# abargum/RAVE

Hardware: AMD Instinct MI355X
Metric: audio samples/sec/GPU (48 kHz v2 encode+decode); × real-time factor (higher is better)
Workload: dtype fp32 (per conv / fused unit the faster of exact-fp32 MFMA and fp32 on the bf16 matrix cores: operands split exactly into 3 bf16 parts (24 significand bits), 6 of the 9 cross products (the 3 dropped are each < 2^-25 |a b|), fp32 accumulate; edges exact-fp32 MFMA); 1 GPU; v2 non-causal encode+decode, 16 x 65536 samples per GPU (BASELINE configs[1]); global_batch=16, samples_per_clip=65536, parallelism=dp1 (batch shards, RCCL all-gather of latents)

## Files before the change

### include/rave_amd.h

```cpp
#ifndef RAVE_AMD_H
#define RAVE_AMD_H

#include <stddef.h>
#include <stdint.h>

#ifdef __cplusplus
extern "C" {
#endif

#define RAVE_ABI_VERSION 21
#define RAVE_SPLITK_TICKETS 4096
#define RAVE_SPLITK_STATUS_WORD (RAVE_SPLITK_TICKETS - 1)

enum {
    RAVE_OK = 0,
    RAVE_ERR_ARG = -1,
    RAVE_ERR_HIP = -2,
    RAVE_ERR_UNSUPPORTED = -3,
    RAVE_ERR_STATE = -4,
    RAVE_ERR_COOP = -5
};

enum { RAVE_ACT_NONE = 0, RAVE_ACT_LEAKY = 1, RAVE_ACT_SNAKE = 2 };

// ... 167 lines not shown

typedef struct rave_noise_backward_args {
    int32_t batch, frames, n_band, noise_bands;
    int32_t target, _pad0;
    const float* amp; int64_t a_sb, a_sc;
    const float* u;   int64_t u_sb;
    const float* gy;  int64_t gy_sb, gy_sc;
    float* gamp;      int64_t ga_sb, ga_sc;
} rave_noise_backward_args;
int rave_noise_synth_backward(const rave_noise_backward_args* a, void* stream);

typedef struct rave_adain_args {
    int32_t batch, channels, t_len, mode;
    int32_t max_batch, row0;
    const float* x; int64_t x_sb, x_sc;
    float* y;       int64_t y_sb, y_sc;
    float* stats;
    float* counters;
    uint32_t* ticket;
} rave_adain_args;
int rave_adain(const rave_adain_args* a, void* stream);

typedef struct rave_adain_backward_args {
    int32_t batch, channels, t_len, mode;
    int32_t max_batch, row0;
    const float* gy; int64_t gy_sb, gy_sc;
    float* gx;       int64_t gx_sb, gx_sc;
    const float* stats;
    const float* counters;
} rave_adain_backward_args;
int rave_adain_backward(const rave_adain_backward_args* a, void* stream);

typedef struct rave_unit_args {
    int32_t channels, batch, t_len, dilation;
    int32_t pad_left, act;
    float leaky_slope; int32_t precision;
    const float* x; int64_t x_sb, x_sc;
    float* y;       int64_t y_sb, y_sc;
    const float* weight;
    const float* bias1; const float* bias2;
    const float* alpha0; const float* alpha2;
    float* workspace;
    uint32_t* status;
    int32_t x_len;
    int32_t res_shift;
    int32_t coop_rb;
    int32_t reserved0;
} rave_unit_args;
int64_t rave_unit_packed_size(int channels);
int rave_unit_pack_weight(const float* w1, const float* w2, int channels, float* packed);
int64_t rave_unit_split_packed_size(int channels);
int rave_unit_split_pack_weight(const float* w1, const float* w2, int channels, float* packed);
int rave_unit_ring_pack_weight(const float* w1, const float* w2, int channels, float* packed);
int64_t rave_unit_bf3_packed_size(int channels);
int rave_unit_bf3_pack_weight(const float* w1, const float* w2, int channels, float* packed);
int64_t rave_unit_workspace(const rave_unit_args* a);
int rave_residual_unit(const rave_unit_args* a, void* stream);
int rave_debug_coop(int64_t spin_limit, int force_giveup);

#define RAVE_STACK_UNITS 3
typedef struct rave_stack_args {
    int32_t channels, batch, t_len, act;
    float leaky_slope; int32_t precision;
    int32_t dilation[RAVE_STACK_UNITS], pad_left[RAVE_STACK_UNITS];
    const float* x; int64_t x_sb, x_sc;
    float* y;       int64_t y_sb, y_sc;
    const float* weight[RAVE_STACK_UNITS];
    const float* bias1[RAVE_STACK_UNITS];
    const float* bias2[RAVE_STACK_UNITS];
    const float* alpha0[RAVE_STACK_UNITS];
    const float* alpha2[RAVE_STACK_UNITS];
} rave_stack_args;
int rave_stack_supported(int channels);
int rave_residual_stack(const rave_stack_args* a, void* stream);

typedef struct rave_edge_args {
    int32_t batch, frames;
    int32_t conv_c_in, conv_c_out, conv_kernel, conv_pad_left;
    int32_t pqmf_taps, pqmf_pad_left;
    int32_t mode, act;
    float leaky_slope;
    int32_t fill_channels, fill_t;
    int32_t precision;
    const float* x;     int64_t x_sb, x_sc;
    float* y;           int64_t y_sb, y_sc;
    const float* weight;
    const float* bias;
    const float* alpha;
    const float* filter;
    const float* noise; int64_t n_sb, n_sc;
    float* fill_y;      int64_t f_sb, f_sc;
    const float* fill_values;
    int64_t fill_vs;
} rave_edge_args;
int rave_encoder_head(const rave_edge_args* a, void* stream);
int rave_decoder_tail(const rave_edge_args* a, void* stream);
#define RAVE_EDGE_FILTER_FLOATS 8836
int rave_encoder_head_pack_filter(const float* hkf, int n_band, int taps, int n_out_bands, float* image);
int rave_decoder_tail_pack_filter(const float* hki, int n_band, int taps, float* image);
int rave_encoder_head_pack_filter_f32(const float* hkf, int n_band, int taps, int n_out_bands, float* image);
int rave_decoder_tail_pack_filter_f32(const float* hki, int n_band, int taps, float* image);

enum {
    RAVE_OP_CONV = 1,
    RAVE_OP_PQMF_ANALYSIS = 2,
    RAVE_OP_PQMF_SYNTHESIS = 3,
    RAVE_OP_FILL = 4,
    RAVE_OP_RVQ_ENCODE = 5,
    RAVE_OP_RVQ_DECODE = 6,
    RAVE_OP_SHIFT_HISTORY = 7,
    RAVE_OP_COPY = 8,
    RAVE_OP_NOISE = 9,
    RAVE_OP_ADAIN = 10,
    RAVE_OP_UNIT = 11,
    RAVE_OP_STACK = 12,
    RAVE_OP_HEAD = 13,
    RAVE_OP_TAIL = 14
};

#define RAVE_OP_PAYLOAD 240
typedef struct rave_plan_op {
    int32_t kind, _pad0;
    union {
        rave_conv1d_args conv;
        rave_pqmf_analysis_args ana;
        rave_pqmf_synthesis_args syn;
        rave_fill_args fill;
        rave_rvq_args rvq;
        rave_shift_args shift;
        rave_copy_args copy;
        rave_noise_args noise;
        rave_adain_args adain;
        rave_unit_args unit;
        rave_stack_args stack;
        rave_edge_args edge;
        unsigned char raw[RAVE_OP_PAYLOAD];
    } u;
} rave_plan_op;

typedef struct rave_reloc {
    int32_t op, field_offset, slot, _pad0;
    int64_t byte_offset;
} rave_reloc;

typedef struct rave_plan rave_plan;
int rave_plan_create(const rave_plan_op* ops, int n_ops, const rave_reloc* relocs, int n_relocs,
                     rave_plan** out);
int rave_plan_run(rave_plan* plan, void* const* slots, int n_slots, void* stream);
int rave_plan_destroy(rave_plan* plan);
int rave_plan_size(const rave_plan* plan);
int rave_plan_profile(rave_plan* plan, int enable);
int rave_plan_op_times(rave_plan* plan, float* ms, int n);

int rave_fill_uniform(float* y, int64_t n, uint64_t seed, float lo, float hi, void* stream);

typedef struct rave_fir_args {
    int32_t batch, t_in, t_out, phases, taps, stride, pad_left, _pad0;
    const float* x; int64_t x_sb;
    float* y;       int64_t y_sb;
    const float* h;
} rave_fir_args;
int rave_fir(const rave_fir_args* a, void* stream);

typedef struct rave_row_stats_args {
    int32_t batch, channels, t_len, act;
    float leaky_slope, var_min, var_max, _pad0;
    const float* x; int64_t x_sb, x_sc;
    float* y;       int64_t y_sb;
} rave_row_stats_args;
int rave_row_stats(const rave_row_stats_args* a, void* stream);

typedef struct rave_attn_pool_args {
    int32_t batch, channels, t_len, act;
    float leaky_slope, var_min, var_max, _pad0;
    const float* x;      int64_t x_sb, x_sc;
    const float* logits; int64_t l_sb, l_sc;
    float* y;            int64_t y_sb;
// ... 196 lines not shown
```

### rave_amd/_native.py

```python
from __future__ import annotations

import ctypes as C
import os

_HERE = os.path.dirname(os.path.abspath(__file__))
LIB_PATH = os.path.join(_HERE, "librave_amd.so")
if os.environ.get("RAVE_AMD_DIAG_LIB") == "1":
    LIB_PATH = os.path.join(_HERE, "librave_amd_diag.so")
if os.environ.get("RAVE_AMD_LIB_VARIANT"):
    LIB_PATH = os.path.join(_HERE, f"librave_amd_{os.environ['RAVE_AMD_LIB_VARIANT']}.so")

RAVE_OK = 0
RAVE_ERR_ARG = -1
RAVE_ERR_HIP = -2
RAVE_ERR_UNSUPPORTED = -3
RAVE_ERR_STATE = -4
RAVE_ERR_COOP = -5

ACT = {"none": 0, "leaky": 1, "snake": 2}

OP_CONV = 1
OP_PQMF_ANALYSIS = 2
OP_PQMF_SYNTHESIS = 3
OP_FILL = 4
# ... 121 lines not shown


class AdainArgs(C.Structure):
    _fields_ = [("batch", i32), ("channels", i32), ("t_len", i32), ("mode", i32),
                ("max_batch", i32), ("row0", i32),
                ("x", vp), ("x_sb", i64), ("x_sc", i64),
                ("y", vp), ("y_sb", i64), ("y_sc", i64),
                ("stats", vp), ("counters", vp), ("ticket", vp)]


class NoiseBackwardArgs(C.Structure):
    _fields_ = [("batch", i32), ("frames", i32), ("n_band", i32), ("noise_bands", i32),
                ("target", i32), ("_pad0", i32),
                ("amp", vp), ("a_sb", i64), ("a_sc", i64),
                ("u", vp), ("u_sb", i64),
                ("gy", vp), ("gy_sb", i64), ("gy_sc", i64),
                ("gamp", vp), ("ga_sb", i64), ("ga_sc", i64)]


class AdainBackwardArgs(C.Structure):
    _fields_ = [("batch", i32), ("channels", i32), ("t_len", i32), ("mode", i32),
                ("max_batch", i32), ("row0", i32),
                ("gy", vp), ("gy_sb", i64), ("gy_sc", i64),
                ("gx", vp), ("gx_sb", i64), ("gx_sc", i64),
                ("stats", vp), ("counters", vp)]


class UnitArgs(C.Structure):
    _fields_ = [("channels", i32), ("batch", i32), ("t_len", i32), ("dilation", i32),
                ("pad_left", i32), ("act", i32), ("leaky_slope", f32), ("precision", i32),
                ("x", vp), ("x_sb", i64), ("x_sc", i64),
                ("y", vp), ("y_sb", i64), ("y_sc", i64),
                ("weight", vp), ("bias1", vp), ("bias2", vp), ("alpha0", vp), ("alpha2", vp),
                ("workspace", vp), ("status", vp), ("x_len", i32), ("res_shift", i32),
                ("coop_rb", i32), ("reserved0", i32)]


STACK_UNITS = 3


class StackArgs(C.Structure):
    _fields_ = ([("channels", i32), ("batch", i32), ("t_len", i32), ("act", i32),
                 ("leaky_slope", f32), ("precision", i32)]
                + [(f"dilation{u}", i32) for u in range(STACK_UNITS)]
                + [(f"pad_left{u}", i32) for u in range(STACK_UNITS)]
                + [("x", vp), ("x_sb", i64), ("x_sc", i64), ("y", vp), ("y_sb", i64), ("y_sc", i64)]
                + [(f"{f}{u}", vp) for f in ("weight", "bias1", "bias2", "alpha0", "alpha2")
                   for u in range(STACK_UNITS)])


class FirArgs(C.Structure):
    _fields_ = [("batch", i32), ("t_in", i32), ("t_out", i32), ("phases", i32), ("taps", i32),
                ("stride", i32), ("pad_left", i32), ("_pad0", i32),
                ("x", vp), ("x_sb", i64), ("y", vp), ("y_sb", i64), ("h", vp)]


class RowStatsArgs(C.Structure):
    _fields_ = [("batch", i32), ("channels", i32), ("t_len", i32), ("act", i32),
                ("leaky_slope", f32), ("var_min", f32), ("var_max", f32), ("_pad0", i32),
                ("x", vp), ("x_sb", i64), ("x_sc", i64), ("y", vp), ("y_sb", i64)]


class AttnPoolArgs(C.Structure):
    _fields_ = [("batch", i32), ("channels", i32), ("t_len", i32), ("act", i32),
                ("leaky_slope", f32), ("var_min", f32), ("var_max", f32), ("_pad0", i32),
                ("x", vp), ("x_sb", i64), ("x_sc", i64), ("logits", vp), ("l_sb", i64), ("l_sc", i64),
                ("y", vp), ("y_sb", i64)]


class LinearArgs(C.Structure):
    _fields_ = [("batch", i32), ("n_in", i32), ("n_out", i32), ("_pad0", i32),
                ("x", vp), ("x_sb", i64), ("w", vp), ("bias", vp), ("y", vp), ("y_sb", i64)]


class MaxPoolArgs(C.Structure):
    _fields_ = [("batch", i32), ("channels", i32), ("t_out", i32), ("kernel", i32),
                ("x", vp), ("x_sb", i64), ("x_sc", i64), ("y", vp), ("y_sb", i64), ("y_sc", i64)]


class EdgeArgs(C.Structure):
    _fields_ = [("batch", i32), ("frames", i32), ("conv_c_in", i32), ("conv_c_out", i32), ("conv_kernel", i32),
                ("conv_pad_left", i32), ("pqmf_taps", i32), ("pqmf_pad_left", i32), ("mode", i32), ("act", i32),
                ("leaky_slope", f32), ("fill_channels", i32), ("fill_t", i32), ("precision", i32),
                ("x", vp), ("x_sb", i64), ("x_sc", i64), ("y", vp), ("y_sb", i64), ("y_sc", i64),
                ("weight", vp), ("bias", vp), ("alpha", vp), ("filter", vp),
                ("noise", vp), ("n_sb", i64), ("n_sc", i64),
                ("fill_y", vp), ("f_sb", i64), ("f_sc", i64), ("fill_values", vp), ("fill_vs", i64)]


STFT_MAX_SCALES = 8


class StftArgs(C.Structure):
    _fields_ = [("rows", i32), ("t_len", i32), ("n", i32), ("_pad0", i32),
                ("x", vp), ("table", vp), ("y", vp)]


class DistanceArgs(C.Structure):
    _fields_ = [("rows", i32), ("t_len", i32), ("n_scales", i32), ("log_epsilon", f32),
                ("scales", i32 * STFT_MAX_SCALES),
                ("x", vp), ("y", vp), ("tables", vp * STFT_MAX_SCALES),
                ("workspace", vp), ("out", vp)]


STFT_LOSS_V1, STFT_LOSS_MULTIRES = 0, 1


class StftLossArgs(C.Structure):
    _fields_ = [("rows", i32), ("t_len", i32), ("n_res", i32), ("kind", i32),
                ("n_fft", i32 * STFT_MAX_SCALES), ("hop", i32 * STFT_MAX_SCALES), ("win", i32 * STFT_MAX_SCALES),
                ("log_epsilon", f32), ("_pad0", i32),
                ("tables", vp * STFT_MAX_SCALES), ("target", vp), ("value", vp),
                ("workspace", vp), ("out", vp), ("saved", vp), ("grad_out", vp), ("grad_value", vp)]


class YinArgs(C.Structure):
    _fields_ = [("rows", i32), ("t_len", i32), ("sample_rate", i32), ("_pad0", i32),
                ("pitch_min", C.c_double), ("pitch_max", C.c_double),
                ("frame_stride", C.c_double), ("threshold", C.c_double),
                ("x_sr", i64), ("x", vp), ("f0", vp), ("cmdf", vp)]


class F0OneHotArgs(C.Structure):
    _fields_ = [("batch", i32), ("frames", i32), ("bins", i32), ("_pad0", i32),
                ("log_lo", f32), ("log_span", f32),
                ("y_sb", i64), ("y_sc", i64), ("f0", vp), ("y", vp)]


MAX_RATIOS = 8
MAX_DILATIONS = 8


class ModelConfig(C.Structure):
    _fields_ = [("n_band", i32), ("enc_bands", i32), ("capacity", i32), ("latent_size", i32),
                ("kernel_size", i32), ("speaker_size", i32), ("n_ratios", i32),
                ("ratios", i32 * MAX_RATIOS), ("n_dilations", i32 * MAX_RATIOS),
                ("dilations", (i32 * MAX_DILATIONS) * MAX_RATIOS),
                ("amplitude_modulation", i32), ("causal", i32), ("activation", i32), ("adain", i32),
                ("leaky_slope", f32), ("conv_bias", i32), ("convt_bias", i32),
                ("noise", i32), ("noise_hidden", i32), ("noise_bands", i32), ("n_noise_ratios", i32),
                ("noise_ratios", i32 * MAX_RATIOS), ("rvq_quantizers", i32), ("rvq_codebook_size", i32),
                ("fuse_units", i32), ("speaker_rows", i32)]


class Param(C.Structure):
    _fields_ = [("name", C.c_char_p), ("data", vp), ("numel", i64)]


class OpInfo(C.Structure):
    _fields_ = [("kind", i32), ("precision", i32), ("flops", C.c_double), ("bytes", C.c_double),
                ("label", C.c_char * 96)]


PAYLOAD = 240


class PlanOp(C.Structure):
    _fields_ = [("kind", i32), ("_pad0", i32), ("raw", C.c_ubyte * PAYLOAD)]


class Reloc(C.Structure):
    _fields_ = [("op", i32), ("field_offset", i32), ("slot", i32), ("_pad0", i32),
                ("byte_offset", i64)]


STRUCTS = [ConvArgs, AnalysisArgs, SynthesisArgs, FillArgs, RvqArgs, ShiftArgs, PlanOp, Reloc,
           CopyArgs, NoiseArgs, AdainArgs, UnitArgs, StackArgs, ModelConfig, Param, OpInfo,
           FirArgs, RowStatsArgs, AttnPoolArgs, LinearArgs, MaxPoolArgs, EdgeArgs,
           StftArgs, DistanceArgs, YinArgs, F0OneHotArgs, SynthesisBackwardArgs, AnalysisBackwardArgs,
           ConvBackwardArgs, NoiseBackwardArgs, AdainBackwardArgs, StftLossArgs]

EXPORTS = [
    "rave_last_error", "rave_abi_version", "rave_struct_sizes",
    "rave_conv1d_chunk", "rave_conv1d_packed_size", "rave_conv1d_pack_weight", "rave_conv1d_pack_weight_device",
    "rave_conv1d",
    "rave_conv1d_workspace", "rave_conv1d_backward_workspace", "rave_conv1d_backward_data",
    "rave_conv1d_backward_weight", "rave_conv_transpose1d_backward_workspace", "rave_conv_transpose1d_backward_data",
    "rave_conv_transpose1d_backward_weight", "rave_conv1d_configs", "rave_conv1d_split_packed_size", "rave_conv1d_split_pack_weight",
    "rave_conv1d_ring_pack_weight", "rave_conv1d_bf3_packed_size", "rave_conv1d_bf3_pack_weight",
    "rave_pqmf_analysis", "rave_pqmf_synthesis", "rave_pqmf_analysis_backward", "rave_pqmf_synthesis_backward",
    "rave_fill_channels", "rave_copy",
    "rave_rvq_workspace", "rave_rvq_encode", "rave_rvq_decode", "rave_shift_history", "rave_noise_synth", "rave_adain",
    "rave_noise_synth_backward", "rave_adain_backward",
    "rave_unit_packed_size", "rave_unit_pack_weight", "rave_residual_unit",
    "rave_unit_split_packed_size", "rave_unit_split_pack_weight", "rave_unit_ring_pack_weight",
    "rave_unit_bf3_packed_size", "rave_unit_bf3_pack_weight",
    "rave_unit_workspace", "rave_debug_coop", "rave_model_check",
    "rave_stack_supported", "rave_residual_stack",
    "rave_plan_create", "rave_plan_run", "rave_plan_destroy", "rave_plan_size",
    "rave_plan_profile", "rave_plan_op_times", "rave_fill_uniform",
    "rave_model_param_count", "rave_model_param_info", "rave_model_create", "rave_model_destroy",
    "rave_model_encode", "rave_model_decode", "rave_model_forward", "rave_model_encode_codes",
    "rave_model_decode_codes", "rave_model_noise_shape", "rave_model_adain_control", "rave_model_set_row0",
    "rave_model_set_speaker", "rave_model_set_speakers", "rave_model_set_speaker_row0", "rave_model_speaker_info",
    "rave_model_adain_count", "rave_model_adain_info", "rave_model_adain_get", "rave_model_adain_set",
    "rave_model_tuning_get", "rave_model_tuning_set", "rave_model_plan_ops", "rave_model_profile",
    "rave_model_op_times", "rave_stream_create", "rave_stream_destroy", "rave_stream_reset",
    "rave_stream_encode", "rave_stream_decode", "rave_stream_encode_codes", "rave_stream_decode_codes",
    "rave_stream_delay",
    "rave_stream_launches",
    "rave_fir", "rave_row_stats", "rave_attn_pool", "rave_linear", "rave_maxpool",
    "rave_encoder_head", "rave_decoder_tail", "rave_encoder_head_pack_filter", "rave_decoder_tail_pack_filter",
    "rave_encoder_head_pack_filter_f32", "rave_decoder_tail_pack_filter_f32",
    "rave_stft_table_size", "rave_stft_pack_table", "rave_stft_mag",
    "rave_audio_distance_workspace", "rave_audio_distance",
    "rave_yin_shape", "rave_yin", "rave_f0_onehot", "rave_pitch_onehot",
    "rave_stft_loss_table_size", "rave_stft_loss_pack_table", "rave_stft_loss_workspace",
    "rave_stft_loss_forward", "rave_stft_loss_backward",
]
EDGE_FILTER_FLOATS = 8836


class NativeError(RuntimeError):
    pass


def _load():
    if not os.path.exists(LIB_PATH):
        raise ImportError(f"rave_amd native library not built: {LIB_PATH} is missing "
                          "(run `python -c 'import __graft_entry__ as g; g.build()'` or "
                          "`make -C rave_amd/csrc`)")
    lib = C.CDLL(LIB_PATH)
    lib.rave_last_error.restype = C.c_char_p
    lib.rave_abi_version.restype = C.c_int
    lib.rave_struct_sizes.argtypes = [C.POINTER(i64), C.c_int]
    lib.rave_conv1d_chunk.argtypes = [C.c_int] * 5
    lib.rave_conv1d_packed_size.argtypes = [C.c_int] * 6
    lib.rave_conv1d_packed_size.restype = i64
    lib.rave_conv1d_pack_weight.argtypes = [vp] + [C.c_int] * 7 + [vp]
    lib.rave_conv1d_pack_weight_device.argtypes = [vp] + [C.c_int] * 7 + [vp, vp]
    lib.rave_conv1d_workspace.argtypes = [C.POINTER(ConvArgs)]
    lib.rave_conv1d_configs.argtypes = [C.POINTER(ConvArgs), C.POINTER(i32), C.c_int]
    lib.rave_conv1d_split_packed_size.argtypes = [C.c_int] * 6
    lib.rave_conv1d_split_packed_size.restype = i64
    lib.rave_conv1d_split_pack_weight.argtypes = [vp] + [C.c_int] * 7 + [vp]
    lib.rave_conv1d_ring_pack_weight.argtypes = [vp] + [C.c_int] * 7 + [vp]
    lib.rave_conv1d_bf3_packed_size.argtypes = [C.c_int] * 6
    lib.rave_conv1d_bf3_packed_size.restype = i64
    lib.rave_conv1d_bf3_pack_weight.argtypes = [vp] + [C.c_int] * 7 + [vp]
    lib.rave_encoder_head_pack_filter.argtypes = [vp, C.c_int, C.c_int, C.c_int, vp]
    lib.rave_encoder_head_pack_filter_f32.argtypes = [vp, C.c_int, C.c_int, C.c_int, vp]
    lib.rave_decoder_tail_pack_filter_f32.argtypes = [vp, C.c_int, C.c_int, vp]
    lib.rave_decoder_tail_pack_filter.argtypes = [vp, C.c_int, C.c_int, vp]
    lib.rave_unit_packed_size.argtypes = [C.c_int]
    lib.rave_unit_packed_size.restype = i64
    lib.rave_unit_pack_weight.argtypes = [vp, vp, C.c_int, vp]
    lib.rave_unit_workspace.argtypes = [C.c_void_p]
    lib.rave_unit_workspace.restype = i64
    lib.rave_debug_coop.argtypes = [i64, C.c_int]
    lib.rave_unit_split_packed_size.argtypes = [C.c_int]
    lib.rave_stack_supported.argtypes = [C.c_int]
    lib.rave_unit_split_packed_size.restype = i64
    lib.rave_unit_split_pack_weight.argtypes = [vp, vp, C.c_int, vp]
    lib.rave_unit_ring_pack_weight.argtypes = [vp, vp, C.c_int, vp]
    lib.rave_unit_bf3_packed_size.argtypes = [C.c_int]
    lib.rave_unit_bf3_packed_size.restype = i64
    lib.rave_unit_bf3_pack_weight.argtypes = [vp, vp, C.c_int, vp]
    lib.rave_conv1d_workspace.restype = i64
    lib.rave_conv1d_backward_workspace.argtypes = [C.POINTER(ConvBackwardArgs)]
    lib.rave_conv1d_backward_workspace.restype = i64
    lib.rave_conv_transpose1d_backward_workspace.argtypes = [C.POINTER(ConvBackwardArgs)]
    lib.rave_conv_transpose1d_backward_workspace.restype = i64
    lib.rave_rvq_workspace.argtypes = [C.POINTER(RvqArgs)]
    lib.rave_rvq_workspace.restype = i64
    for name, st in [("rave_conv1d", ConvArgs), ("rave_pqmf_analysis", AnalysisArgs),
                     ("rave_pqmf_synthesis", SynthesisArgs), ("rave_fill_channels", FillArgs),
                     ("rave_pqmf_synthesis_backward", SynthesisBackwardArgs),
                     ("rave_pqmf_analysis_backward", AnalysisBackwardArgs),
                     ("rave_conv1d_backward_data", ConvBackwardArgs),
                     ("rave_conv1d_backward_weight", ConvBackwardArgs),
                     ("rave_conv_transpose1d_backward_data", ConvBackwardArgs),
                     ("rave_conv_transpose1d_backward_weight", ConvBackwardArgs),
                     ("rave_rvq_encode", RvqArgs), ("rave_rvq_decode", RvqArgs),
                     ("rave_shift_history", ShiftArgs), ("rave_copy", CopyArgs),
                     ("rave_noise_synth", NoiseArgs), ("rave_adain", AdainArgs),
                     ("rave_noise_synth_backward", NoiseBackwardArgs), ("rave_adain_backward", AdainBackwardArgs),
                     ("rave_residual_unit", UnitArgs), ("rave_residual_stack", StackArgs),
                     ("rave_fir", FirArgs), ("rave_row_stats", RowStatsArgs), ("rave_attn_pool", AttnPoolArgs),
                     ("rave_linear", LinearArgs), ("rave_maxpool", MaxPoolArgs),
                     ("rave_encoder_head", EdgeArgs), ("rave_decoder_tail", EdgeArgs)]:
        getattr(lib, name).argtypes = [C.POINTER(st), vp]
    lib.rave_stft_table_size.argtypes = [C.c_int]
    lib.rave_stft_table_size.restype = i64
    lib.rave_stft_pack_table.argtypes = [C.c_int, vp]
    lib.rave_stft_mag.argtypes = [C.POINTER(StftArgs), vp]
    lib.rave_audio_distance_workspace.argtypes = [C.POINTER(DistanceArgs)]
    lib.rave_audio_distance_workspace.restype = i64
    lib.rave_audio_distance.argtypes = [C.POINTER(DistanceArgs), vp]
    lib.rave_stft_loss_table_size.argtypes = [C.c_int, C.c_int]
    lib.rave_stft_loss_table_size.restype = i64
    lib.rave_stft_loss_pack_table.argtypes = [C.c_int, C.c_int, vp]
    lib.rave_stft_loss_workspace.argtypes = [C.POINTER(StftLossArgs)]
    lib.rave_stft_loss_workspace.restype = i64
# ... 222 lines not shown
```

### rave_amd/csrc/edge_split.hip

```cpp
#include "common.h"
#include "pack_shared.h"

#include <algorithm>
#include <cmath>

namespace rave {

typedef _Float16 e_h8 __attribute__((ext_vector_type(8)));
typedef _Float16 e_h4 __attribute__((ext_vector_type(4)));
typedef float e_f32x4 __attribute__((ext_vector_type(4)));
typedef float e_f32x16 __attribute__((ext_vector_type(16)));
typedef float e_f32x8 __attribute__((ext_vector_type(8)));
typedef __bf16 e_b8 __attribute__((ext_vector_type(8)));
typedef __bf16 e_b4 __attribute__((ext_vector_type(4)));

__device__ __forceinline__ e_f32x8 e_ld8(const float* p) {
    const e_f32x4 u = *reinterpret_cast<const e_f32x4*>(p), v = *reinterpret_cast<const e_f32x4*>(p + 4);
    return e_f32x8{u[0], u[1], u[2], u[3], v[0], v[1], v[2], v[3]};
}

constexpr int kEdgeWaves = 8;
constexpr int kEdgeNT = 64 * kEdgeWaves;
constexpr int kEdgeK7 = 7;
constexpr int kEdgeKW = 544;
constexpr int kEdgeFP = 552;
constexpr int kSynTapsE = 33;
constexpr int kAnaTapsE = 513;

constexpr int kEdgeFilterHalves = 2 * 16 * kEdgeFP;
constexpr int kEdgeFilterFloats = kEdgeFilterHalves / 2 + 4;

struct EdgeGeo {
    int tiles;
    int w_mb;
    int w_bytes;
    int y_vec;
    int64_t w_frag_floats;
};

__device__ __forceinline__ void e_split(float v, _Float16& hi, _Float16& lo) {
    hi = (_Float16)v;
    lo = (_Float16)((v - (float)hi) * 2048.0f);
}

struct EdgeW {
    __amdgpu_buffer_rsrc_t rs;
    int mb_count;
    int np = 2;
    __device__ unsigned off(int chunk, int mb, int tap, int plane, int lane) const {
        return (unsigned)((((chunk * mb_count + mb) * kEdgeK7 + tap) * np + plane) * 1024 + lane * 16);
    }
    __device__ e_h8 frag(int chunk, int mb, int tap, int plane, int lane) const {
        return __builtin_bit_cast(e_h8, __builtin_amdgcn_raw_buffer_load_b128(rs, off(chunk, mb, tap, plane, lane), 0, 0));
    }
    __device__ static e_f32x8 f32(const e_h8& p0, const e_h8& p1) {
        const e_f32x4 u = __builtin_bit_cast(e_f32x4, p0), v = __builtin_bit_cast(e_f32x4, p1);
        return e_f32x8{u[0], u[1], u[2], u[3], v[0], v[1], v[2], v[3]};
    }
};

#ifdef RAVE_EDGE_STOP
#define EDGE_STOP(n, v)                                                   \
    if (RAVE_EDGE_STOP == (n)) {                                          \
        if (threadIdx.x == 0) a.y[(int64_t)blockIdx.x] = (float)(v);      \
        return;                                                           \
    }
#else
#define EDGE_STOP(n, v)
#endif

constexpr int kHF = 256;
constexpr int kHAB = kHF / 32 + 1;
constexpr int kHBR = 32 * kHAB;
constexpr int kHBP = 24;
constexpr int kHXS = 512 * (kHAB - 1) + 32 * 15 + kEdgeKW;
__host__ __device__ constexpr int e_xi(int i) { return i + 8 * (i >> 7); }
constexpr int kHXP = e_xi(kHXS) + 8;
constexpr int kHeadLds = (2 * 16 * kEdgeFP + 2 * kHXP + 2 * kHBR * kHBP) * 2 + 4 * kEdgeWaves * 4 + 16 +
                         kEdgeWaves * 64 * 4 * 4;
constexpr int kHeadBaBand = (3 * 16 * kEdgeFP + 3 * kHXP) * 2;
static_assert(kHeadBaBand % 16 == 0, "band planes 16-byte aligned");
constexpr int kHeadLdsBa = kHeadBaBand + kHBR * kHBP * 4 + 4 * kEdgeWaves * 4 + 16 + kEdgeWaves * 64 * 4 * 4;

template <int AR>
__global__ __launch_bounds__(kEdgeNT) void encoder_head_kernel(rave_edge_args a, EdgeGeo geo) {
    constexpr bool FC = AR != 0;
    constexpr bool F32 = AR == 1, BA = AR == 2;
// ... 245 lines not shown
    const int MB = (a.conv_c_out + 31) / 32;
    e_h8 wr[kEdgeK7][2][2];
#pragma unroll
    for (int q = 0; q < kEdgeK7; ++q)
#pragma unroll
        for (int j = 0; j < 2; ++j)
#pragma unroll
            for (int pl = 0; pl < 2; ++pl) wr[q][j][pl] = j < MB ? W.frag(0, j, q, pl, lane) : e_h8{};
    put_bands(wave, v0, 1.f);
    if (extra) put_bands(wave + kEdgeWaves, v1, 1.f);
    if constexpr (AR == 0) vote_cast(vote + 8, wave, bmax);
    __syncthreads();
    float bs = 1.f;
    if (AR == 0 && __builtin_expect(vote_any<kEdgeWaves>(vote + 8), 0)) {
        bs = ldexpf(1.f, -__builtin_amdgcn_readfirstlane(split_shift(block_max<kEdgeWaves>(bmax, red))));
        put_bands(wave, v0, bs);
        if (extra) put_bands(wave + kEdgeWaves, v1, bs);
        __syncthreads();
    }
    EDGE_STOP(2, bh[tid] + bl[tid])

    const int h = lane >> 5, l32 = lane & 31;
    e_f32x16 acc[2];
#pragma unroll
    for (int j = 0; j < 2; ++j)
#pragma unroll
        for (int r = 0; r < 16; ++r) acc[j][r] = 0.f;
#pragma unroll
    for (int q = 0; q < kEdgeK7; ++q) {
        const int row = 32 * wave + l32 + q;
        if constexpr (FC) {
            const e_f32x8 x8 = e_ld8(bf + row * kHBP);
#pragma unroll
            for (int j = 0; j < 2; ++j) {
                if (j >= MB) break;
                const e_f32x8 w8 = EdgeW::f32(wr[q][j][0], wr[q][j][1]);
#pragma unroll
                for (int e = 0; e < 4; ++e) {
                    if (2 * e >= a.conv_c_in) break;
                    const float w_odd = __shfl(w8[2 * e + 1], l32);
                    const float wv = h ? w_odd : w8[2 * e];
                    const float xv = h ? x8[2 * e + 1] : x8[2 * e];
                    acc[j] = __builtin_amdgcn_mfma_f32_32x32x2f32(xv, wv, acc[j], 0, 0, 0);
                }
            }
            continue;
        }
        const e_h8 xh8 = *reinterpret_cast<const e_h8*>(bh + row * kHBP + 8 * h);
        const e_h8 xl8 = *reinterpret_cast<const e_h8*>(bl + row * kHBP + 8 * h);
#pragma unroll
        for (int j = 0; j < 2; ++j) {
            if (j >= MB) break;
            const e_h8 b2 = wr[q][j][0] * (_Float16)2048.0f;
            acc[j] = __builtin_amdgcn_mfma_f32_32x32x16_f16(xh8, b2, acc[j], 0, 0, 0);
            acc[j] = __builtin_amdgcn_mfma_f32_32x32x16_f16(xl8, wr[q][j][0], acc[j], 0, 0, 0);
            acc[j] = __builtin_amdgcn_mfma_f32_32x32x16_f16(xh8, wr[q][j][1], acc[j], 0, 0, 0);
        }
    }
    EDGE_STOP(3, acc[0][0] + acc[1][7])
    const float* rsc = a.weight + geo.w_frag_floats;
    const float inv_bs = 1.0f / bs;
    float* yb = a.y + (int64_t)b * a.y_sb;
#pragma unroll
    for (int j = 0; j < 2; ++j) {
        if (j >= MB) break;
        const int m = 32 * j + l32;
        if (m >= a.conv_c_out) continue;
        const float rs = rsc[m] * inv_bs;
        const float bias = a.bias ? a.bias[m] : 0.f;
#pragma unroll
        for (int c4 = 0; c4 < 4; ++c4) {
            const int t = n0 + 32 * wave + 8 * c4 + 4 * h;
            e_f32x4 v;
#pragma unroll
            for (int e = 0; e < 4; ++e) v[e] = acc[j][4 * c4 + e] * rs + bias;
            float* dst = yb + (int64_t)m * a.y_sc + t;
            if (t + 3 < F && geo.y_vec) {
                *reinterpret_cast<e_f32x4*>(dst) = v;
            } else {
#pragma unroll
                for (int e = 0; e < 4; ++e)
                    if (t + e < F) dst[e] = v[e];
            }
        }
    }
}

constexpr int kTF = 256;
constexpr int kTB = (kTF + kSynTapsE + 31) / 32;
constexpr int kTC = 64;
constexpr int kTXR = 32 * kTB + kEdgeK7 - 1;
constexpr int kTXP = kTC + 8;
constexpr int kTSW = kTF + kSynTapsE + 1;
constexpr int kTSP = 24;
constexpr int kTPlane = 2 * kTXR * kTXP;
static_assert(2 * kTSW * kTSP <= kTPlane, "synthesis planes reuse the act(x) planes");
constexpr int kTailLds = (2 * 16 * kEdgeFP + kTPlane) * 2 + 2 * kEdgeWaves * 4 + 16;
constexpr int kTailBfX = 3 * kTXR * kTXP * 2;
constexpr int kTailLdsBf = kTailBfX + 2 * kEdgeWaves * 4 + 16;
constexpr int kTailBsFilt = 75776;
static_assert(kTailBsFilt >= 3 * kTSW * kTSP * 2 + kEdgeWaves * 16 * 64 * 4 &&
              kTailBsFilt + 3 * 16 * kEdgeFP * 2 <= kTailBfX, "bf16x3 synthesis LDS reuse");

template <bool SNAKE, bool AM, int AR>
__global__ __launch_bounds__(kEdgeNT) void decoder_tail_kernel(rave_edge_args a, EdgeGeo geo) {
    constexpr bool F32 = AR == 1, BF = AR == 2;
    const int tiles = geo.tiles;
    extern __shared__ __attribute__((aligned(16))) char e_smem[];
    _Float16* fh = reinterpret_cast<_Float16*>(e_smem);
    _Float16* fl = fh + 16 * kEdgeFP;
    _Float16* xh = BF ? fh : fl + 16 * kEdgeFP;
    _Float16* xl = xh + kTXR * kTXP;
    _Float16* xm = xl + kTXR * kTXP;
    _Float16* sh = xh;
    _Float16* sl = xh + kTSW * kTSP;
    float* red = reinterpret_cast<float*>(BF ? reinterpret_cast<char*>(e_smem) + kTailBfX
                                             : reinterpret_cast<char*>(xh + kTPlane));
    float* ff = reinterpret_cast<float*>(e_smem);
    float* xf = reinterpret_cast<float*>(xh);
    float* sf = xf;
    __bf16* sbh = reinterpret_cast<__bf16*>(xh);
    __bf16* sbl = sbh + kTSW * kTSP;
    __bf16* sbm = sbl + kTSW * kTSP;
    __bf16* fbh = reinterpret_cast<__bf16*>(e_smem + kTailBsFilt);
    __bf16* fbm = fbh + 16 * kEdgeFP;
    __bf16* fbl = fbm + 16 * kEdgeFP;
    const int tid = threadIdx.x, lane = tid & 63;
    const int wave = __builtin_amdgcn_readfirstlane(tid >> 6);
    const int nmain = tiles * a.batch;
    const int lg = __builtin_amdgcn_readfirstlane(xcd_major(blockIdx.x, nmain));
    const int b = lg / tiles;
    const int n0 = (lg - b * tiles) * kTF;
    const int F = a.frames;
    const int f0 = n0 - a.pqmf_pad_left;
    const int x0 = f0 - a.conv_pad_left;
    const float slope = a.leaky_slope;

    unsigned char* vote = reinterpret_cast<unsigned char*>(red + 2 * kEdgeWaves);
    constexpr int NPW = BF ? 3 : 2;
    const EdgeW W{make_rsrc(a.weight, (int64_t)geo.w_bytes), geo.w_mb, NPW};
    constexpr int KS = (kTC / 16) * kEdgeK7;
    constexpr int RING = 4;
    e_h8 wr[RING][NPW];
#pragma unroll
    for (int s = 0; s < RING; ++s)
#pragma unroll
        for (int pl = 0; pl < NPW; ++pl) wr[s][pl] = W.frag(s / kEdgeK7, 0, s % kEdgeK7, pl, lane);
    constexpr int FQ = (kEdgeFilterHalves / 8 + kEdgeNT - 1) / kEdgeNT;
    e_h8 fq[BF ? FQ : 1];
    if constexpr (BF) {
        const e_h8* src = reinterpret_cast<const e_h8*>(a.filter);
#pragma unroll
        for (int i = 0; i < FQ; ++i) {
            const int k = tid + i * kEdgeNT;
            if (k < kEdgeFilterHalves / 8) fq[i] = src[k];
        }
    } else {
        const e_h8* src = reinterpret_cast<const e_h8*>(a.filter);
        e_h8* dst = reinterpret_cast<e_h8*>(fh);
        for (int i = tid; i < kEdgeFilterHalves / 8; i += kEdgeNT) dst[i] = src[i];
    }
    const float f_unscale = a.filter[kEdgeFilterHalves / 2];
    constexpr int NG = kTC / 4;
    constexpr int XT = (NG * kTXR + kEdgeNT - 1) / kEdgeNT;
    const float* xb = a.x + (int64_t)b * a.x_sb;
    e_f32x4 xv[XT];
// ... 274 lines not shown
static int edge_lds_attr(K kern, int lds, bool& done) {
    if (!done) {
        RAVE_CHECK_HIP(hipFuncSetAttribute(reinterpret_cast<const void*>(kern),
                                           hipFuncAttributeMaxDynamicSharedMemorySize, lds));
        done = true;
    }
    return RAVE_OK;
}

template <typename Fn>
static void edge_filter_image(Fn&& A, float* image, bool f32) {
    if (f32) {
        for (int r = 0; r < 16; ++r)
            for (int k = 0; k < kEdgeFP; ++k) image[r * kEdgeFP + k] = k < kEdgeKW ? A(r, k) : 0.f;
        image[kEdgeFilterHalves / 2] = 1.f;
        for (int i = kEdgeFilterHalves / 2 + 1; i < kEdgeFilterFloats; ++i) image[i] = 0.f;
        return;
    }
    double amax = 0.0;
    for (int r = 0; r < 16; ++r)
        for (int k = 0; k < kEdgeKW; ++k) amax = std::max(amax, std::fabs((double)A(r, k)));
    const int e = row_exponent(amax);
    _Float16* hi = reinterpret_cast<_Float16*>(image);
    _Float16* lo = hi + 16 * kEdgeFP;
    for (int r = 0; r < 16; ++r)
        for (int k = 0; k < kEdgeFP; ++k) {
            const float v = k < kEdgeKW ? (float)std::ldexp((double)A(r, k), e) : 0.f;
            split_f16(v, hi[r * kEdgeFP + k], lo[r * kEdgeFP + k]);
        }
    image[kEdgeFilterHalves / 2] = (float)std::ldexp(1.0, -(e + 11));
    for (int i = kEdgeFilterHalves / 2 + 1; i < kEdgeFilterFloats; ++i) image[i] = 0.f;
}

static int head_pack(const float* hkf, int n_band, int taps, int n_out_bands, float* image, bool f32) {
    RAVE_CHECK_ARG(hkf && image, "encoder_head_pack_filter: null pointer");
    if (n_band != 16 || taps != kAnaTapsE || n_out_bands < 1 || n_out_bands > 8) {
        set_error("encoder_head_pack_filter: built for 16 bands, 513 taps, <= 8 output bands");
        return RAVE_ERR_UNSUPPORTED;
    }
    edge_filter_image([&](int r, int j) -> float {
        const int p = r >> 3, k = r & 7, jj = j - 16 * p;
        return (k < n_out_bands && jj >= 0 && jj < taps) ? hkf[(int64_t)k * taps + jj] : 0.f;
    }, image, f32);
    return RAVE_OK;
}
extern "C" int rave_encoder_head_pack_filter(const float* hkf, int n_band, int taps, int n_out_bands, float* image) {
    return head_pack(hkf, n_band, taps, n_out_bands, image, false);
}
extern "C" int rave_encoder_head_pack_filter_f32(const float* hkf, int n_band, int taps, int n_out_bands,
                                                 float* image) {
    return head_pack(hkf, n_band, taps, n_out_bands, image, true);
}

static int tail_pack(const float* hki, int n_band, int taps, float* image, bool f32) {
    RAVE_CHECK_ARG(hki && image, "decoder_tail_pack_filter: null pointer");
    if (n_band != 16 || taps != kSynTapsE) {
        set_error("decoder_tail_pack_filter: built for 16 bands, 33 taps");
        return RAVE_ERR_UNSUPPORTED;
    }
    edge_filter_image([&](int m, int k) -> float {
        const int tap = k >> 4, c = k & 15;
        return tap < taps ? hki[((int64_t)m * n_band + c) * taps + tap] : 0.f;
    }, image, f32);
    return RAVE_OK;
}
extern "C" int rave_decoder_tail_pack_filter(const float* hki, int n_band, int taps, float* image) {
    return tail_pack(hki, n_band, taps, image, false);
}
extern "C" int rave_decoder_tail_pack_filter_f32(const float* hki, int n_band, int taps, float* image) {
    return tail_pack(hki, n_band, taps, image, true);
}

static int edge_prec(const rave_edge_args& a, bool& f32, bool allow_bf3 = false) {
    f32 = a.precision == RAVE_PREC_F32_RING;
    if (a.precision != 0 && a.precision != RAVE_PREC_SPLIT16 && !f32 &&
        !(allow_bf3 && a.precision == RAVE_PREC_BF16X3)) {
        set_error(allow_bf3 ? "edge: precision must be RAVE_PREC_SPLIT16, RAVE_PREC_F32_RING or RAVE_PREC_BF16X3"
                            : "edge: precision must be RAVE_PREC_SPLIT16 or RAVE_PREC_F32_RING");
        return RAVE_ERR_ARG;
    }
    return RAVE_OK;
}

extern "C" int rave_encoder_head(const rave_edge_args* p, void* stream) {
    RAVE_CHECK_ARG(p && p->x && p->y && p->weight && p->filter, "encoder_head: null pointer");
    const rave_edge_args& a = *p;
    RAVE_CHECK_ARG(a.batch > 0 && a.frames > 0, "encoder_head: empty shape");
    if (a.conv_kernel != kEdgeK7 || a.conv_c_in < 1 || a.conv_c_in > 8 || a.conv_c_out < 1 || a.conv_c_out > 64 ||
        a.conv_pad_left < 0 || a.conv_pad_left > kEdgeK7 - 1 || a.pqmf_taps != kAnaTapsE) {
        set_error("encoder_head: built for RAVE's 513-tap analysis, <= 8 bands and a 7-tap conv to <= 64 channels");
        return RAVE_ERR_UNSUPPORTED;
    }
    RAVE_CHECK_ARG(a.fill_channels == 0 || (a.fill_y && a.fill_values && a.fill_t > 0),
                   "encoder_head: fill needs fill_y, fill_values and fill_t");
    RAVE_CHECK_ARG(a.fill_channels == 0 || a.fill_vs == 0 || a.fill_vs >= a.fill_channels,
                   "encoder_head: fill_vs must be 0 (one shared vector) or >= fill_channels");
    if (a.act != RAVE_ACT_NONE) {
        set_error("encoder_head: the fused analysis + first conv applies no input activation (act must be RAVE_ACT_NONE)");
        return RAVE_ERR_UNSUPPORTED;
    }
    bool f32;
    int rc = edge_prec(a, f32, true);
    if (rc != RAVE_OK) return rc;
    const int ar = a.precision == RAVE_PREC_BF16X3 ? 2 : f32 ? 1 : 0;
    const EdgeGeo g = edge_geometry(a, kHF);
    static bool attr[3] = {false, false, false};
    auto kern = ar == 2 ? encoder_head_kernel<2> : ar == 1 ? encoder_head_kernel<1> : encoder_head_kernel<0>;
    const int lds = ar == 2 ? kHeadLdsBa : kHeadLds;
    rc = edge_lds_attr(kern, lds, attr[ar]);
    if (rc != RAVE_OK) return rc;
    const int grid = g.tiles * a.batch;
    launch(kern, dim3(grid), dim3(kEdgeNT), (uint32_t)lds, as_stream(stream), a, g);
    return launch_status("encoder_head_kernel");
}

extern "C" int rave_decoder_tail(const rave_edge_args* p, void* stream) {
    RAVE_CHECK_ARG(p && p->x && p->y && p->weight && p->filter, "decoder_tail: null pointer");
    const rave_edge_args& a = *p;
    RAVE_CHECK_ARG(a.batch > 0 && a.frames > 0, "decoder_tail: empty shape");
    if (a.conv_kernel != kEdgeK7 || a.conv_c_in != kTC || (a.conv_c_out != 16 && a.conv_c_out != 32) ||
        a.conv_pad_left < 0 || a.conv_pad_left > kEdgeK7 - 1 || a.pqmf_taps != kSynTapsE ||
        (a.mode != 1 && a.mode != 2) || (a.mode == 1) != (a.conv_c_out == 32)) {
        set_error("decoder_tail: built for a 7-tap conv 64 -> 32 (amplitude modulation) or 64 -> 16 "
                  "into RAVE's 33-tap synthesis");
        return RAVE_ERR_UNSUPPORTED;
    }
    RAVE_CHECK_ARG(a.act == RAVE_ACT_LEAKY || (a.act == RAVE_ACT_SNAKE && a.alpha),
                   "decoder_tail: act must be RAVE_ACT_LEAKY or RAVE_ACT_SNAKE (with alpha)");
    RAVE_CHECK_ARG(reinterpret_cast<uintptr_t>(a.y) % 16 == 0 && a.y_sb % 4 == 0,
                   "decoder_tail: output must be 16-byte aligned");
    bool f32;
    int rc = edge_prec(a, f32, true);
    if (rc != RAVE_OK) return rc;
    const bool bf = a.precision == RAVE_PREC_BF16X3;
    const int ar = bf ? 2 : f32 ? 1 : 0;
    const EdgeGeo g = edge_geometry(a, kTF, bf ? 3 : 2);
    const dim3 grid(g.tiles * a.batch);
    const bool snake = a.act == RAVE_ACT_SNAKE, am = a.mode == 1;
    auto pick = [&](auto art) {
        constexpr int AR = decltype(art)::value;
        return snake ? (am ? decoder_tail_kernel<true, true, AR> : decoder_tail_kernel<true, false, AR>)
                     : (am ? decoder_tail_kernel<false, true, AR> : decoder_tail_kernel<false, false, AR>);
    };
    auto kern = ar == 2 ? pick(IC<2>{}) : ar == 1 ? pick(IC<1>{}) : pick(IC<0>{});
    const int lds = bf ? kTailLdsBf : kTailLds;
    static bool attr[12] = {false, false, false, false, false, false, false, false, false, false, false, false};
    rc = edge_lds_attr(kern, lds, attr[4 * ar + 2 * snake + am]);
    if (rc != RAVE_OK) return rc;
    launch(kern, grid, dim3(kEdgeNT), (uint32_t)lds, as_stream(stream), a, g);
    return launch_status("decoder_tail_kernel");
}
```

Before: 1.411 billion samples/s.

## Add paired-band bf16x3 encoder head kernel with smaller tiles as default

Adds a new encoder_head_pair_kernel for the bf16x3 precision path with at most 6 bands. It uses 128-frame tiles and packs two frame rows per MFMA column, so that two workgroups fit on a CU. The halo block is split across waves 4-7 with a partial-sum reduction. It becomes the default (AUTO) unless RAVE_EDGE_FORM=1, and the edge args struct gains a form field. The aim is better occupancy and less wasted MFMA work on the PQMF analysis, at the cost of more tiles and more redundant halo input loads.

```diff
diff --git a/include/rave_amd.h b/include/rave_amd.h
--- a/include/rave_amd.h
+++ b/include/rave_amd.h
@@ -273,6 +273,8 @@
     float leaky_slope;
     int32_t fill_channels, fill_t;
     int32_t precision;
+    int32_t form;
+    int32_t _pad0;
     const float* x;     int64_t x_sb, x_sc;
     float* y;           int64_t y_sb, y_sc;
     const float* weight;
@@ -284,6 +286,7 @@
     const float* fill_values;
     int64_t fill_vs;
 } rave_edge_args;
+enum { RAVE_EDGE_FORM_AUTO = 0, RAVE_EDGE_FORM_WIDE = 1, RAVE_EDGE_FORM_PAIR = 2 };
 int rave_encoder_head(const rave_edge_args* a, void* stream);
 int rave_decoder_tail(const rave_edge_args* a, void* stream);
 #define RAVE_EDGE_FILTER_FLOATS 8836
diff --git a/rave_amd/_native.py b/rave_amd/_native.py
--- a/rave_amd/_native.py
+++ b/rave_amd/_native.py
@@ -227,6 +227,7 @@
     _fields_ = [("batch", i32), ("frames", i32), ("conv_c_in", i32), ("conv_c_out", i32), ("conv_kernel", i32),
                 ("conv_pad_left", i32), ("pqmf_taps", i32), ("pqmf_pad_left", i32), ("mode", i32), ("act", i32),
                 ("leaky_slope", f32), ("fill_channels", i32), ("fill_t", i32), ("precision", i32),
+                ("form", i32), ("_pad0", i32),
                 ("x", vp), ("x_sb", i64), ("x_sc", i64), ("y", vp), ("y_sb", i64), ("y_sc", i64),
                 ("weight", vp), ("bias", vp), ("alpha", vp), ("filter", vp),
                 ("noise", vp), ("n_sb", i64), ("n_sc", i64),
@@ -354,6 +355,7 @@
     "rave_stft_loss_forward", "rave_stft_loss_backward",
 ]
 EDGE_FILTER_FLOATS = 8836
+EDGE_FORM_AUTO, EDGE_FORM_WIDE, EDGE_FORM_PAIR = 0, 1, 2
 
 
 class NativeError(RuntimeError):
diff --git a/rave_amd/csrc/edge_split.hip b/rave_amd/csrc/edge_split.hip
--- a/rave_amd/csrc/edge_split.hip
+++ b/rave_amd/csrc/edge_split.hip
@@ -3,6 +3,7 @@
 
 #include <algorithm>
 #include <cmath>
+#include <cstdlib>
 
 namespace rave {
 
@@ -414,6 +415,201 @@
                 for (int e = 0; e < 4; ++e)
                     if (t + e < F) dst[e] = v[e];
             }
+        }
+    }
+}
+
+constexpr int kH2F = 128;
+constexpr int kH2AB = kH2F / 32 + 1;
+constexpr int kH2BR = kH2F + 8;
+constexpr int kH2FR = 12;
+constexpr int kH2XS = 512 * (kH2AB - 1) + 32 * 15 + kEdgeKW;
+constexpr int kH2XP = e_xi(kH2XS) + 8;
+constexpr int kHead2Band = (3 * kH2FR * kEdgeFP + 3 * kH2XP) * 2;
+static_assert(kH2XS % kEdgeNT == 0 && kHead2Band % 16 == 0 && (kH2XP * 2) % 16 == 0, "paired head layout");
+constexpr int kHead2Lds = kHead2Band + kH2BR * kHBP * 4 + kEdgeWaves * 64 * 4 * 4;
+static_assert(kHead2Lds <= 80 * 1024, "two workgroups to a CU");
+static_assert(kH2AB - 1 == kEdgeWaves / 2, "waves 0-3 whole blocks, waves 4-7 the halo block");
+
+__global__ __launch_bounds__(kEdgeNT) void encoder_head_pair_kernel(rave_edge_args a, EdgeGeo geo) {
+    const int tiles = geo.tiles;
+    extern __shared__ __attribute__((aligned(16))) char e_smem[];
+    __bf16* gbh = reinterpret_cast<__bf16*>(e_smem);
+    __bf16* gbm = gbh + kH2FR * kEdgeFP;
+    __bf16* gbl = gbm + kH2FR * kEdgeFP;
+    __bf16* wbh = gbl + kH2FR * kEdgeFP;
+    __bf16* wbm = wbh + kH2XP;
+    __bf16* wbl = wbm + kH2XP;
+    float* bf = reinterpret_cast<float*>(e_smem + kHead2Band);
+    float* part = bf + kH2BR * kHBP;
+    const int tid = threadIdx.x, lane = tid & 63;
+    const int wave = __builtin_amdgcn_readfirstlane(tid >> 6);
+    const int nmain = tiles * a.batch;
+    const int lg = __builtin_amdgcn_readfirstlane(xcd_major(blockIdx.x, nmain));
+    const int b = lg / tiles;
+    const int tile = lg - b * tiles;
+    const int n0 = tile * kH2F;
+    const bool odd = tile & 1;
+    if (a.fill_channels > 0) {
+        float* z = a.fill_y + (int64_t)b * a.f_sb;
+        const float* fv = a.fill_values + (int64_t)b * a.fill_vs;
+        const int n = a.fill_channels * a.fill_t;
+        for (int i = tile * kEdgeNT + tid; i < n; i += tiles * kEdgeNT) {
+            const int c = i / a.fill_t, t = i - c * a.fill_t;
+            z[(int64_t)c * a.f_sc + t] = fv[c];
+        }
+    }
+    const int F = a.frames;
+    const int T = F * 16;
+    const int g0 = n0 - a.conv_pad_left;
+    const int s0 = 16 * g0 - a.pqmf_pad_left;
+
+    constexpr int XT = kH2XS / kEdgeNT;
+    const float* xb = a.x + (int64_t)b * a.x_sb;
+    float xv[XT];
+#pragma unroll
+    for (int it = 0; it < XT; ++it) {
+        const int t = s0 + tid + it * kEdgeNT;
+        const float v = xb[min(max(t, 0), T - 1)];
+        xv[it] = (t >= 0 && t < T) ? v : 0.f;
+    }
+    {
+        constexpr int RP = kEdgeFP / 4;
+        const e_f32x4* src = reinterpret_cast<const e_f32x4*>(a.filter);
+        for (int i = tid; i < kH2FR * RP; i += kEdgeNT) {
+            e_b4 hi, mid, lo;
+            bf3_split_pk(src[i + (i >= 6 * RP ? 2 * RP : 0)], hi, mid, lo);
+            *reinterpret_cast<e_b4*>(gbh + 4 * i) = hi;
+            *reinterpret_cast<e_b4*>(gbm + 4 * i) = mid;
+            *reinterpret_cast<e_b4*>(gbl + 4 * i) = lo;
+        }
+    }
+#pragma unroll
+    for (int it = 0; it < XT; ++it) {
+        const int i = tid + it * kEdgeNT;
+        const float v = xv[it];
+        const __bf16 hi = (__bf16)v;
+        const float r = v - (float)hi;
+        const __bf16 mid = (__bf16)r;
+        wbh[e_xi(i)] = hi;
+        wbm[e_xi(i)] = mid;
+        wbl[e_xi(i)] = (__bf16)(r - (float)mid);
+    }
+    const EdgeW W{make_rsrc(a.weight, (int64_t)geo.w_bytes), geo.w_mb};
+    const int MB = (a.conv_c_out + 31) / 32;
+    const int cb = wave & 3, j = wave >> 2;
+    e_h8 wr[kEdgeK7][2];
+#pragma unroll
+    for (int q = 0; q < kEdgeK7; ++q)
+#pragma unroll
+        for (int pl = 0; pl < 2; ++pl) wr[q][pl] = j < MB ? W.frag(0, j, q, pl, lane) : e_h8{};
+    __syncthreads();
+    EDGE_STOP(1, (float)wbh[tid] + (float)gbh[tid])
+
+    const int g = lane >> 4, col = lane & 15;
+    const int frow = 6 * (col >> 3) + min(col & 7, 5);
+    auto ba_step = [&](int blk, int s, e_f32x4& c) __attribute__((always_inline)) {
+        const int ka = frow * kEdgeFP + 32 * s + 8 * g;
+        const int xi = e_xi(512 * blk + 32 * col + 32 * s + 8 * g);
+        const e_b8 fh8 = *reinterpret_cast<const e_b8*>(gbh + ka), fm8 = *reinterpret_cast<const e_b8*>(gbm + ka),
+                   fl8 = *reinterpret_cast<const e_b8*>(gbl + ka);
+        const e_b8 xh8 = *reinterpret_cast<const e_b8*>(wbh + xi), xm8 = *reinterpret_cast<const e_b8*>(wbm + xi),
+                   xl8 = *reinterpret_cast<const e_b8*>(wbl + xi);
+        c = __builtin_amdgcn_mfma_f32_16x16x32_bf16(fl8, xh8, c, 0, 0, 0);
+        c = __builtin_amdgcn_mfma_f32_16x16x32_bf16(fh8, xl8, c, 0, 0, 0);
+        c = __builtin_amdgcn_mfma_f32_16x16x32_bf16(fm8, xm8, c, 0, 0, 0);
+        c = __builtin_amdgcn_mfma_f32_16x16x32_bf16(fm8, xh8, c, 0, 0, 0);
+        c = __builtin_amdgcn_mfma_f32_16x16x32_bf16(fh8, xm8, c, 0, 0, 0);
+        c = __builtin_amdgcn_mfma_f32_16x16x32_bf16(fh8, xh8, c, 0, 0, 0);
+    };
+    auto chain = [&](int blk, int first, int stride) __attribute__((always_inline)) {
+        e_f32x4 c = {0.f, 0.f, 0.f, 0.f};
+        for (int s = first; s < kEdgeKW / 32; s += stride) ba_step(blk, s, c);
+        return c;
+    };
+    const float unscale = a.filter[kEdgeFilterHalves / 2];
+    auto put_bands = [&](int blk, const e_f32x4& acc) __attribute__((always_inline)) {
+        const int p = g >> 1;
+        const int row = 32 * blk + 2 * col + p;
+        const int f = g0 + row;
+        const bool fok = f >= 0 && f < F;
+        e_f32x4 v;
+#pragma unroll
+        for (int r = 0; r < 4; ++r) {
+            const int k = 4 * (g & 1) + r;
+            float x = acc[r] * unscale;
+            if ((k & 1) && !(f & 1)) x = -x;
+            v[r] = (fok && k < 6) ? x : 0.f;
+        }
+        if (row < kH2BR) *reinterpret_cast<e_f32x4*>(bf + row * kHBP + 4 * (g & 1)) = v;
+    };
+    const int halo = kH2AB - 1;
+    if (wave < halo) {
+        e_f32x4 c0 = {0.f, 0.f, 0.f, 0.f}, c1 = c0;
+#pragma unroll
+        for (int s = 0; s < kEdgeKW / 32; ++s) ba_step(wave, s, (s & 1) ? c1 : c0);
+        put_bands(wave, c0 + c1);
+    } else {
+        const int w4 = wave - halo;
+        if (odd) {
+            e_f32x4 pa = chain(halo, w4, kEdgeWaves), pb = chain(halo, w4 + 4, kEdgeWaves);
+            const e_f32x4 z4 = {0.f, 0.f, 0.f, 0.f};
+            pa = (pa + z4) + z4;
+            pb = (pb + z4) + z4;
+            *reinterpret_cast<e_f32x4*>(part + (w4 * 64 + lane) * 4) = pa;
+            *reinterpret_cast<e_f32x4*>(part + ((w4 + 4) * 64 + lane) * 4) = pb;
+        } else if (w4 < 2) {
+            *reinterpret_cast<e_f32x4*>(part + (w4 * 64 + lane) * 4) = chain(halo, w4, 2);
+        }
+    }
+    __syncthreads();
+    if (wave == halo) {
+        e_f32x4 acc1 = *reinterpret_cast<const e_f32x4*>(part + lane * 4);
+        const int np = odd ? kEdgeWaves : 2;
+        for (int w2 = 1; w2 < np; ++w2) acc1 += *reinterpret_cast<const e_f32x4*>(part + (w2 * 64 + lane) * 4);
+        put_bands(halo, acc1);
+    }
+    __syncthreads();
+    EDGE_STOP(2, bf[tid])
+
+    const int h = lane >> 5, l32 = lane & 31;
+    if (j >= MB) return;
+    e_f32x16 acc;
+#pragma unroll
+    for (int r = 0; r < 16; ++r) acc[r] = 0.f;
+#pragma unroll
+    for (int q = 0; q < kEdgeK7; ++q) {
+        const int row = 32 * cb + l32 + q;
+        const e_f32x8 x8 = e_ld8(bf + row * kHBP);
+        const e_f32x8 w8 = EdgeW::f32(wr[q][0], wr[q][1]);
+#pragma unroll
+        for (int e = 0; e < 4; ++e) {
+            if (2 * e >= a.conv_c_in) break;
+            const float w_odd = __shfl(w8[2 * e + 1], l32);
+            const float wv = h ? w_odd : w8[2 * e];
+            const float xe = h ? x8[2 * e + 1] : x8[2 * e];
+            acc = __builtin_amdgcn_mfma_f32_32x32x2f32(xe, wv, acc, 0, 0, 0);
+        }
+    }
+    EDGE_STOP(3, acc[0] + acc[7])
+    const int m = 32 * j + l32;
+    if (m >= a.conv_c_out) return;
+    const float rs = (a.weight + geo.w_frag_floats)[m];
+    const float bias = a.bias ? a.bias[m] : 0.f;
+    float* yb = a.y + (int64_t)b * a.y_sb;
+#pragma unroll
+    for (int c4 = 0; c4 < 4; ++c4) {
+        const int t = n0 + 32 * cb + 8 * c4 + 4 * h;
+        e_f32x4 v;
+#pragma unroll
+        for (int e = 0; e < 4; ++e) v[e] = acc[4 * c4 + e] * rs + bias;
+        float* dst = yb + (int64_t)m * a.y_sc + t;
+        if (t + 3 < F && geo.y_vec) {
+            *reinterpret_cast<e_f32x4*>(dst) = v;
+        } else {
+#pragma unroll
+            for (int e = 0; e < 4; ++e)
+                if (t + e < F) dst[e] = v[e];
         }
     }
 }
@@ -854,6 +1050,14 @@
     return RAVE_OK;
 }
 
+static bool edge_form_wide() {
+    static const bool wide = [] {
+        const char* e = std::getenv("RAVE_EDGE_FORM");
+        return e && e[0] == '1';
+    }();
+    return wide;
+}
+
 extern "C" int rave_encoder_head(const rave_edge_args* p, void* stream) {
     RAVE_CHECK_ARG(p && p->x && p->y && p->weight && p->filter, "encoder_head: null pointer");
     const rave_edge_args& a = *p;
@@ -875,6 +1079,20 @@
     int rc = edge_prec(a, f32, true);
     if (rc != RAVE_OK) return rc;
     const int ar = a.precision == RAVE_PREC_BF16X3 ? 2 : f32 ? 1 : 0;
+    RAVE_CHECK_ARG(a.form >= RAVE_EDGE_FORM_AUTO && a.form <= RAVE_EDGE_FORM_PAIR, "encoder_head: form must be RAVE_EDGE_FORM_*");
+    const bool pair_ok = ar == 2 && a.conv_c_in <= 6;
+    if (a.form == RAVE_EDGE_FORM_PAIR && !pair_ok) {
+        set_error("encoder_head: RAVE_EDGE_FORM_PAIR is the bf16x3 head's, for <= 6 bands");
+        return RAVE_ERR_UNSUPPORTED;
+    }
+    if (a.form == RAVE_EDGE_FORM_PAIR || (a.form == RAVE_EDGE_FORM_AUTO && pair_ok && !edge_form_wide())) {
+        const EdgeGeo g = edge_geometry(a, kH2F);
+        static bool attr2 = false;
+        rc = edge_lds_attr(encoder_head_pair_kernel, kHead2Lds, attr2);
+        if (rc != RAVE_OK) return rc;
+        launch(encoder_head_pair_kernel, dim3(g.tiles * a.batch), dim3(kEdgeNT), (uint32_t)kHead2Lds, as_stream(stream), a, g);
+        return launch_status("encoder_head_pair_kernel");
+    }
     const EdgeGeo g = edge_geometry(a, kHF);
     static bool attr[3] = {false, false, false};
     auto kern = ar == 2 ? encoder_head_kernel<2> : ar == 1 ? encoder_head_kernel<1> : encoder_head_kernel<0>;
@@ -901,6 +1119,11 @@
                    "decoder_tail: act must be RAVE_ACT_LEAKY or RAVE_ACT_SNAKE (with alpha)");
     RAVE_CHECK_ARG(reinterpret_cast<uintptr_t>(a.y) % 16 == 0 && a.y_sb % 4 == 0,
                    "decoder_tail: output must be 16-byte aligned");
+    RAVE_CHECK_ARG(a.form >= RAVE_EDGE_FORM_AUTO && a.form <= RAVE_EDGE_FORM_PAIR, "decoder_tail: form must be RAVE_EDGE_FORM_*");
+    if (a.form == RAVE_EDGE_FORM_PAIR) {
+        set_error("decoder_tail: RAVE_EDGE_FORM_PAIR is the bf16x3 head's; the tail has the wide form only");
+        return RAVE_ERR_UNSUPPORTED;
+    }
     bool f32;
     int rc = edge_prec(a, f32, true);
     if (rc != RAVE_OK) return rc;
```

Result: no change. 1.419 billion samples/s, median of 6 (+0.6%).
